# nianticlabs/simplerecon

Hardware: AMD Instinct MI355X
Metric: depth frames/sec (640x480, 7 src views, 64 planes) (higher is better)
Workload: dtype f32

## Files before the change

### include/simplerecon_hip.h

```cpp
#ifndef SIMPLERECON_HIP_H_
#define SIMPLERECON_HIP_H_

#include <stddef.h>
#include <stdint.h>

#ifdef __cplusplus
extern "C" {
#endif

#define SR_OK 0
#define SR_ERR_INVALID_ARGUMENT 1
#define SR_ERR_UNSUPPORTED 2
#define SR_ERR_WORKSPACE_TOO_SMALL 3
#define SR_ERR_HIP_BASE 1000

enum {
  SR_OPT_MLP_SPLIT = 0, SR_OPT_WINO_SPLIT, SR_OPT_WINO_XCD, SR_OPT_WINO_NT, SR_OPT_WINO_KSPLIT, SR_OPT_CONV_WINO,
  SR_OPT_CONV_TILE, SR_OPT_CONV_KSPLIT, SR_OPT_PW_NT, SR_OPT_PW_KS, SR_OPT_PT_CFG, SR_OPT_PT_KS, SR_OPT_DOT_LDS,
  SR_OPT_DOT_LDS_G, SR_OPT_DOT_LDS_CULL, SR_OPT_DOT_LDS_CAP, SR_OPT_UPSAMPLE_QUAD, SR_OPT_POOL_STREAM,
  SR_OPT_MLP_TILE,
  SR_OPT_COUNT
};
int sr_option_count(void);
const char* sr_option_name(int id);
int sr_option_id(const char* name);
int sr_option_get(int id, int* value);
int sr_option_set(int id, int value, int* previous );
int sr_option_default(int id, int* value);

int sr_abi_version(void);

const char* sr_target_arch(void);


size_t sr_volume_workspace_bytes(int B, int K, int C, int h, int w);

int sr_volume_prepare(const float* src, const float* K_src, const float* T_src_cur,
                      const float* T_cur_src, int B, int K, int C, int h, int w, void* workspace,
                      size_t workspace_bytes, void* stream);

int sr_dot_volume_sweep(const float* cur, const float* invK_cur, const float* planes, int64_t ps_b,
                        int64_t ps_d, int64_t ps_y, int64_t ps_x, int B, int K, int C, int h, int w,
                        int D, float* out_cv, int64_t cv_sb, int64_t cv_sd, int64_t cv_sp,
                        float* out_lowest, uint8_t* out_mask, void* workspace,
                        size_t workspace_bytes, void* stream);

int sr_conv3x3_wino_io_nhwc_fwd(const void* in, int64_t in_batch_stride, int in_pix_stride, const float* packed_u,
                                const float* bias, const void* residual, int64_t res_batch_stride, int res_pix_stride,
                                void* out, int64_t out_batch_stride, int out_pix_stride, int B, int H, int W, int Cin,
                                int Cout, float leaky_slope, int io_dtype, void* stream);
int sr_pw_conv_io_nhwc_fwd(const void* in, int64_t in_batch_stride, int in_pix_stride, const float* packed_w,
                           const float* bias, const void* residual, int64_t res_batch_stride, int res_pix_stride, void* out,
                           int64_t out_batch_stride, int out_pix_stride, int B, int HW, int Cin, int Cout, float act_code,
                           int io_dtype, void* stream);

size_t sr_pw_conv_tiled_workspace_bytes(int M, int Cin, int Cout);
int sr_pw_conv_tiled_plan(int M, int Cin, int Cout, int can_split, int* cfg, int* ks);
int sr_pw_conv_tiled_nhwc_fwd(const float* in, int in_pix_stride, const float* packed_w, const float* bias,
                              const float* gate, const float* residual, int res_pix_stride, float* out,
                              int out_pix_stride, int M, int HW, int Cin, int Cout, float act_code, void* workspace,
                              size_t workspace_bytes, void* stream);
int sr_pw_conv_supported(int Cin, int Cout);
int sr_pw_conv_plan(int B, int HW, int Cin, int Cout, int* nt, int* ks);
int sr_pw_conv_nhwc_fwd(const float* in, int64_t in_batch_stride, int in_pix_stride, const float* packed_w,
                        const float* bias, const float* gate, const float* residual, int64_t res_batch_stride,
                        int res_pix_stride, float* out, int64_t out_batch_stride, int out_pix_stride, int B, int HW,
                        int Cin, int Cout, float act_code, void* stream);

int sr_backproject_fwd(const float* depth, const float* invK, float* out_points, int B, int h, int w, void* stream);
int sr_project3d_fwd(const float* points, const float* K, const float* T, float* out, int B, int N, float eps,
                     void* stream);
int sr_backproject_bwd(const float* grad_points, const float* invK, float* grad_depth, int B, int h, int w, void* stream);
int sr_project3d_bwd(const float* grad_out, const float* points, const float* K, const float* T, float* grad_points, int B,
                     int N, float eps, void* stream);
int sr_pose_distance_fwd(const float* T, float* out, int n, void* stream);
int sr_camera_rays_fwd(const float* points, const float* T, float* out, int B, int N, int in_camera_frame, void* stream);

int sr_selftest_rcp(const float* x, float* out_fast, float* out_div, int n, void* stream);

int sr_dot_volume_fwd(const float* cur, const float* src, const float* K_src,
                      const float* T_src_cur, const float* invK_cur, const float* planes,
                      int64_t ps_b, int64_t ps_d, int64_t ps_y, int64_t ps_x, int B, int K, int C,
                      int h, int w, int D, float* out_cv, int64_t cv_sb, int64_t cv_sd,
                      int64_t cv_sp, float* out_lowest, uint8_t* out_mask, void* workspace,
                      size_t workspace_bytes, void* stream);

int sr_warp_features_fwd(const float* src, const float* K_src, const float* T_src_cur,
                         const float* invK_cur, const float* planes, int64_t ps_b, int64_t ps_d,
                         int64_t ps_y, int64_t ps_x, int B, int K, int C, int h, int w, int Dp,
                         float* out_world, float* out_depths, float* out_warped, float* out_mask,
                         float* out_pix, void* workspace, size_t workspace_bytes, void* stream);

size_t sr_mlp_volume_workspace_bytes(int B, int K, int C, int h, int w, int hidden);

int sr_mlp_pack_weights(const float* W1, const float* b1, const float* W2, const float* b2,
                        const float* W3, const float* b3, int hidden, int B, int K, int C, int h, int w,
                        void* workspace, size_t workspace_bytes, void* stream);

int sr_mlp_volume_sweep(const float* cur, const float* invK_cur, const float* planes, int64_t ps_b,
                        int64_t ps_d, int64_t ps_y, int64_t ps_x, float leaky_slope, int B, int K,
                        int C, int h, int w, int D, float* out_cv, int64_t cv_sb, int64_t cv_sd,
                        int64_t cv_sp, float* out_lowest, uint8_t* out_mask, void* workspace,
                        size_t workspace_bytes, void* stream);

int sr_mlp_volume_tile_shape(int h, int w, int* th, int* tw);

int sr_mlp_volume_fwd(const float* cur, const float* src, const float* K_src, const float* T_src_cur,
                      const float* T_cur_src, const float* invK_cur, const float* planes, int64_t ps_b,
                      int64_t ps_d, int64_t ps_y, int64_t ps_x, const float* W1, const float* b1,
                      const float* W2, const float* b2, const float* W3, const float* b3, int hidden,
                      float leaky_slope, int B, int K, int C, int h, int w, int D, float* out_cv,
                      int64_t cv_sb, int64_t cv_sd, int64_t cv_sp, float* out_lowest, uint8_t* out_mask,
                      int reserve_cus, void* workspace, size_t workspace_bytes, void* stream);


size_t sr_conv_packed_weight_floats(int Cout, int Cin, int ksize);

int sr_conv_pack_weights(const float* weight, int Cout, int Cin, int ksize, float* packed, void* stream);

int sr_conv2d_nhwc_fwd(const float* in, int64_t in_batch_stride, int in_pix_stride,
                       const float* packed_weight, const float* bias, const float* residual,
                       int64_t res_batch_stride, int res_pix_stride, float* out,
                       int64_t out_batch_stride, int out_pix_stride, int B, int H, int W, int Cin,
                       int Cout, int ksize, int stride, float leaky_slope, void* stream);

int sr_conv2d_replicate_nhwc_fwd(const float* in, int64_t in_batch_stride, int in_pix_stride,
                                 const float* packed_weight, const float* bias, const float* residual,
                                 int64_t res_batch_stride, int res_pix_stride, float* out,
                                 int64_t out_batch_stride, int out_pix_stride, int B, int H, int W, int Cin,
                                 int Cout, int ksize, int stride, float leaky_slope, void* stream);

#define SR_ACT_NONE (-1.0f)
#define SR_ACT_SILU (-2.0f)
int sr_conv2d_padded_nhwc_fwd(const float* in, int64_t in_batch_stride, int in_pix_stride,
                              const float* packed_weight, const float* bias, const float* residual,
                              int64_t res_batch_stride, int res_pix_stride, float* out,
                              int64_t out_batch_stride, int out_pix_stride, int B, int H, int W, int Cin,
                              int Cout, int ksize, int stride, int pad_top, int pad_left, int pad_bottom,
                              int pad_right, float leaky_slope, void* stream);

size_t sr_conv_splitk_workspace_bytes(int B, int H, int W, int Cin, int Cout, int ksize, int stride);
int sr_conv2d_splitk_nhwc_fwd(const float* in, int64_t in_batch_stride, int in_pix_stride,
                              const float* packed_weight, const float* bias, const float* residual,
                              int64_t res_batch_stride, int res_pix_stride, float* out,
                              int64_t out_batch_stride, int out_pix_stride, int B, int H, int W, int Cin,
                              int Cout, int ksize, int stride, float leaky_slope, void* workspace,
                              size_t workspace_bytes, void* stream);

size_t sr_wino_packed_weight_floats(int Cout, int Cin);
int sr_wino_pack_weights(const float* weight, int Cout, int Cin, float* packed, void* stream);
int sr_conv_prefers_wino(int B, int H, int W, int Cin, int Cout, int ksize, int stride);
int sr_conv3x3_wino_nhwc_fwd(const float* in, int64_t in_batch_stride, int in_pix_stride,
                             const float* packed_u, const float* bias, const float* residual,
                             int64_t res_batch_stride, int res_pix_stride, float* out,
                             int64_t out_batch_stride, int out_pix_stride, int B, int H, int W, int Cin,
                             int Cout, float leaky_slope, void* stream);

size_t sr_wino4_packed_weight_floats(int Cout, int Cin);
// ... 383 lines not shown
```

### simplerecon_amd/_lib.py

```python
import contextlib
import ctypes as C
import os

import torch

_HERE = os.path.dirname(os.path.abspath(__file__))
LIB_PATH = os.environ.get("SR_HIP_LIBRARY") or os.path.join(_HERE, "libsimplerecon_hip.so")
ABI_VERSION = 3

_lib = None

_p = C.c_void_p
_i = C.c_int
_i64 = C.c_int64
_f = C.c_float
_sz = C.c_size_t

SIGNATURES = {
    "sr_abi_version": (_i, []),
    "sr_option_count": (_i, []),
    "sr_option_name": (C.c_char_p, [_i]),
    "sr_option_id": (_i, [C.c_char_p]),
    "sr_option_get": (_i, [_i, C.POINTER(C.c_int)]),
    "sr_option_set": (_i, [_i, _i, C.POINTER(C.c_int)]),
    "sr_option_default": (_i, [_i, C.POINTER(C.c_int)]),
    "sr_target_arch": (C.c_char_p, []),
    "sr_volume_workspace_bytes": (_sz, [_i, _i, _i, _i, _i]),
    "sr_volume_prepare": (_i, [_p, _p, _p, _p, _i, _i, _i, _i, _i, _p, _sz, _p]),
    "sr_dot_volume_sweep": (_i, [_p, _p, _p, _i64, _i64, _i64, _i64, _i, _i, _i, _i, _i, _i,
                                 _p, _i64, _i64, _i64, _p, _p, _p, _sz, _p]),
    "sr_dot_volume_fwd": (_i, [_p, _p, _p, _p, _p, _p, _i64, _i64, _i64, _i64, _i, _i, _i, _i, _i, _i,
                               _p, _i64, _i64, _i64, _p, _p, _p, _sz, _p]),
    "sr_rgb_stem3x3s2_fwd": (_i, [_p, _i64, _i64, _i64, _i64, _p, _p, _p, _i64, _i, _i, _i, _i, _i, _i, _i, _i, _i, _f, _p]),
    "sr_se_gate2_fwd": (_i, [_p, _i, _i, _p, _p, _p, _p, _p, _p, _i, _i, _i, _p]),
    "sr_conv3x3_wino_io_nhwc_fwd": (_i, [_p, _i64, _i, _p, _p, _p, _i64, _i, _p, _i64, _i, _i, _i, _i, _i, _i, _f, _i, _p]),
    "sr_pw_conv_io_nhwc_fwd": (_i, [_p, _i64, _i, _p, _p, _p, _i64, _i, _p, _i64, _i, _i, _i, _i, _i, _f, _i, _p]),
    "sr_conv16_packed_weight_bytes": (_sz, [_i, _i, _i]),
    "sr_conv16_pack_weights": (_i, [_p, _i, _i, _i, _i, _p, _p]),
    "sr_conv16_supported": (_i, [_i, _i, _i, _i, _i, _i, _i]),
    "sr_conv16_prefers": (_i, [_i, _i, _i, _i, _i, _i, _i]),
    "sr_conv16_nhwc_fwd": (_i, [_p, _i64, _i, _p, _p, _p, _i64, _i, _p, _i64, _i, _i, _i, _i, _i, _i, _i, _i, _f, _i, _i, _p]),
    "sr_conv16_wgrad_supported": (_i, [_i, _i, _i, _i, _i, _i, _i]),
    "sr_conv16_wgrad_prefers": (_i, [_i, _i, _i, _i, _i, _i, _i]),
    "sr_conv16_wgrad_workspace_bytes": (_sz, [_i, _i, _i, _i, _i, _i, _i]),
    "sr_conv16_wgrad_nhwc": (_i, [_p, _i64, _i, _p, _i64, _i, _p, _i, _i, _i, _i, _i, _i, _i, _i, _p, _sz, _p]),
    "sr_act_bwd_bias16_workspace_bytes": (_sz, [_i64, _i]),
    "sr_act_bwd_bias16_nhwc": (_i, [_p, _i, _p, _p, _p, _i64, _i, _f, _i, _p, _sz, _p]),
    "sr_pw_conv_tiled_workspace_bytes": (_sz, [_i, _i, _i]),
    "sr_pw_conv_tiled_plan": (_i, [_i, _i, _i, _i, _p, _p]),
    "sr_pw_conv_tiled_nhwc_fwd": (_i, [_p, _i, _p, _p, _p, _p, _i, _p, _i, _i, _i, _i, _i, _f, _p, _sz, _p]),
    "sr_pw_conv_supported": (_i, [_i, _i]),
    "sr_pw_conv_plan": (_i, [_i, _i, _i, _i, _p, _p]),
    "sr_pw_conv_nhwc_fwd": (_i, [_p, _i64, _i, _p, _p, _p, _p, _i64, _i, _p, _i64, _i, _i, _i, _i, _i, _f, _p]),
    "sr_backproject_fwd": (_i, [_p, _p, _p, _i, _i, _i, _p]),
    "sr_project3d_fwd": (_i, [_p, _p, _p, _p, _i, _i, _f, _p]),
    "sr_backproject_bwd": (_i, [_p, _p, _p, _i, _i, _i, _p]),
    "sr_project3d_bwd": (_i, [_p, _p, _p, _p, _p, _i, _i, _f, _p]),
    "sr_pose_distance_fwd": (_i, [_p, _p, _i, _p]),
    "sr_camera_rays_fwd": (_i, [_p, _p, _p, _i, _i, _i, _p]),
    "sr_selftest_rcp": (_i, [_p, _p, _p, _i, _p]),
    "sr_warp_features_fwd": (_i, [_p, _p, _p, _p, _p, _i64, _i64, _i64, _i64, _i, _i, _i, _i, _i, _i,
                                  _p, _p, _p, _p, _p, _p, _sz, _p]),
    "sr_mlp_volume_workspace_bytes": (_sz, [_i, _i, _i, _i, _i, _i]),
    "sr_mlp_pack_weights": (_i, [_p, _p, _p, _p, _p, _p, _i, _i, _i, _i, _i, _i, _p, _sz, _p]),
    "sr_mlp_volume_sweep": (_i, [_p, _p, _p, _i64, _i64, _i64, _i64, _f, _i, _i, _i, _i, _i, _i,
                                 _p, _i64, _i64, _i64, _p, _p, _p, _sz, _p]),
    "sr_mlp_volume_tile_shape": (_i, [_i, _i, C.POINTER(C.c_int), C.POINTER(C.c_int)]),
    "sr_mlp_volume_fwd": (_i, [_p, _p, _p, _p, _p, _p, _p, _i64, _i64, _i64, _i64, _p, _p, _p, _p, _p, _p, _i,
                               _f, _i, _i, _i, _i, _i, _i, _p, _i64, _i64, _i64, _p, _p, _i, _p, _sz, _p]),
    "sr_conv_packed_weight_floats": (_sz, [_i, _i, _i]),
    "sr_conv_pack_weights": (_i, [_p, _i, _i, _i, _p, _p]),
    "sr_conv2d_nhwc_fwd": (_i, [_p, _i64, _i, _p, _p, _p, _i64, _i, _p, _i64, _i, _i, _i, _i, _i, _i, _i, _i, _f, _p]),
    "sr_conv2d_replicate_nhwc_fwd": (_i, [_p, _i64, _i, _p, _p, _p, _i64, _i, _p, _i64, _i, _i, _i, _i, _i, _i, _i, _i,
                                          _f, _p]),
    "sr_conv2d_padded_nhwc_fwd": (_i, [_p, _i64, _i, _p, _p, _p, _i64, _i, _p, _i64, _i, _i, _i, _i, _i, _i, _i, _i,
                                       _i, _i, _i, _i, _f, _p]),
    "sr_dwconv3x3_pool_bands": (_i, [_i]),
    "sr_dwconv3x3_nhwc_fwd": (_i, [_p, _i64, _i, _p, _p, _p, _i64, _i, _p, _i, _i, _i, _i, _i, _i, _i, _i, _i, _f,
                                   _p]),
    "sr_add_nhwc_fwd": (_i, [_p, _i64, _i, _p, _i64, _i, _p, _i64, _i, _i, _i, _i, _i, _p]),
    "sr_se_scale_nhwc_fwd": (_i, [_p, _i, _p, _p, _p, _p, _p, _p, _i64, _i, _p, _i64, _i, _p, _i, _i, _i, _i, _i,
                                  _p]),
    "sr_se_gate_fwd": (_i, [_p, _i, _i, _p, _p, _p, _p, _p, _i, _i, _i, _p]),
    "sr_scale_channels_nhwc_fwd": (_i, [_p, _i64, _i, _p, _p, _i64, _i, _i, _i, _i, _i, _p]),
    "sr_dot_volume_bwd_scratch_bytes": (_sz, [_i, _i, _i, _i, _i]),
    "sr_dot_volume_bwd": (_i, [_p, _i64, _i64, _i64, _p, _p, _p, _i64, _i64, _i64, _i64, _i, _i, _i, _i, _i, _i, _p, _p,
                               _p, _sz, _p, _sz, _p]),
    "sr_mlp_volume_bwd_scratch_bytes": (_sz, [_i, _i, _i, _i, _i, _i]),
    "sr_mlp_volume_bwd": (_i, [_p, _i64, _i64, _i64, _p, _p, _p, _i64, _i64, _i64, _i64, _p, _p, _p, _p, _p, _f, _i, _i,
                               _i, _i, _i, _i, _i, _p, _p, _p, _p, _p, _p, _p, _p, _p, _sz, _p, _sz, _p]),
    "sr_conv_wgrad_workspace_bytes": (_sz, [_i, _i, _i, _i, _i, _i, _i]),
    "sr_conv_wgrad_nhwc": (_i, [_p, _i64, _i, _p, _i64, _i, _p, _i, _i, _i, _i, _i, _i, _i, _p, _sz, _p]),
    "sr_bias_grad_nhwc": (_i, [_p, _i64, _i, _p, _i, _i, _i, _i, _p]),
    "sr_act_bwd": (_i, [_p, _p, _p, _i64, _f, _p]),
    "sr_act_bwd_bias_workspace_bytes": (_sz, [_i64, _i]),
    "sr_act_bwd_bias_nhwc": (_i, [_p, _p, _p, _p, _i64, _i, _f, _p, _sz, _p]),
    "sr_zero_stuff2x_nhwc": (_i, [_p, _i64, _i, _p, _i, _i, _i, _i, _i, _i, _p]),
    "sr_upsample2x_bwd_nhwc": (_i, [_p, _i64, _i, _p, _i64, _i, _i, _i, _i, _i, _p]),
    "sr_conv_flip_transpose_weights": (_i, [_p, _i, _i, _i, _p, _p]),
    "sr_mul_fwd": (_i, [_p, _p, _p, _i64, _p]),
    "sr_norm_workspace_bytes": (_sz, [_i, _i, _i, _i]),
    "sr_norm_stats_nhwc": (_i, [_p, _i64, _i, _i, _i, _i, _i, _p, _p, _p, _sz, _p]),
    "sr_norm_act_fwd_nhwc": (_i, [_p, _i64, _i, _p, _p, _f, _p, _p, _f, _i, _p, _i64, _i, _i, _i, _i, _p]),
    "sr_norm_act_bwd_nhwc": (_i, [_p, _i64, _i, _p, _i64, _i, _p, _p, _f, _p, _p, _f, _i, _i, _p, _i64, _i, _p, _p,
                                  _i, _i, _i, _p, _sz, _p]),
    "sr_rowsum_nhwc": (_i, [_p, _i64, _i, _p, _i64, _i, _i, _i, _i, _f, _p, _p, _sz, _p]),
    "sr_maxblurpool_bwd_workspace_bytes": (_sz, [_i, _i, _i, _i]),
    "sr_maxblurpool_bwd_nhwc": (_i, [_p, _i64, _i, _p, _i64, _i, _p, _i64, _i, _i, _i, _i, _i, _p, _sz, _p]),
    "sr_replicate_pad_nhwc_fwd": (_i, [_p, _i64, _i, _p, _i, _i, _i, _i, _i, _p]),
    "sr_replicate_pad_nhwc_bwd": (_i, [_p, _p, _i, _i, _i, _i, _i, _p]),
    "sr_im2col7x7s2_nhwc": (_i, [_p, _i64, _i64, _i64, _i64, _p, _i, _i, _i, _i, _p]),
    "sr_dwconv3x3_bwd_workspace_bytes": (_sz, [_i, _i, _i, _i]),
    "sr_dwconv3x3_bwd_nhwc": (_i, [_p, _i64, _i, _p, _i64, _i, _p, _p, _p, _i, _i, _i, _i, _i, _i, _i, _i, _i, _p, _sz,
                                   _p]),
    "sr_scale_bwd_nhwc": (_i, [_p, _i64, _i, _p, _p, _f, _p, _i, _i, _i, _p]),
    "sr_small_linear_fwd": (_i, [_p, _p, _p, _p, _p, _i, _i, _i, _f, _p]),
    "sr_small_linear_bwd": (_i, [_p, _p, _p, _p, _p, _p, _p, _i, _i, _i, _f, _p]),
    "sr_act_in_bwd": (_i, [_p, _p, _p, _i64, _f, _p]),
    "sr_add_act_fwd": (_i, [_p, _p, _p, _p, _i64, _f, _p]),
    "sr_conv_wgrad_padded_workspace_bytes": (_sz, [_i, _i, _i, _i, _i, _i]),
# ... 287 lines not shown
```

### simplerecon_amd/csrc/sr_mlp_volume.hip

```cpp
#include <stdlib.h>
#include <string.h>

#include "sr_buffer.h"
#include "sr_view.h"

#define SR_HID 128
#define SR_VIEW_SLOTS 24
#define SR_INV_FIXED 20
#define SR_PLANE_CHUNK 8

static inline int sr_mlp_steps_var(int K) { return (SR_VIEW_SLOTS / 2) * K; }
static inline int sr_mlp_steps_inv(int K) { return (SR_INV_FIXED + 3 * K + 1) / 2; }
static inline int sr_mlp_steps1(int K) { return sr_mlp_steps_var(K) + sr_mlp_steps_inv(K); }
#define SR_MLP_STEPS2 65

static inline size_t sr_mlp_packed_floats(int K) { return (size_t)(sr_mlp_steps1(K) + SR_MLP_STEPS2) * 256 + 128 + 4; }

__global__ void sr_mlp_pack_kernel(const float* __restrict__ W1, const float* __restrict__ b1,
                                   const float* __restrict__ W2, const float* __restrict__ b2,
                                   const float* __restrict__ W3, const float* __restrict__ b3,
                                   float* __restrict__ packed, int K, int C) {
  const int steps_var = (SR_VIEW_SLOTS / 2) * K;
  const int steps1 = steps_var + (SR_INV_FIXED + 3 * K + 1) / 2;
  const int Cin = C * (K + 1) + 10 * K + 4;
// ... 16 lines not shown
        else if (s == 18) col = o_dot + k;
        else if (s == 19) col = o_ang + k;
        else if (s < 23) col = o_sray + 3 * k + (s - 20);
        else col = (k == 0) ? o_d : -1;
      } else {
        const int u = 2 * (t - steps_var) + (lane >> 5);
        if (u < 16) col = o_cur + u;
        else if (u < 19) col = o_cray + (u - 16);
        else if (u == 19) col = -2;
        else if (u < SR_INV_FIXED + 3 * K) {
          const int k = (u - SR_INV_FIXED) / 3, i = (u - SR_INV_FIXED) - 3 * k;
          col = (i == 0 ? o_pd : (i == 1 ? o_rm : o_tm)) + k;
        }
      }
      v = (col >= 0) ? W1[(size_t)row * Cin + col] : (col == -2 ? b1[row] : 0.0f);
    } else if (e < (steps1 + SR_MLP_STEPS2) * 256) {
      const int e2 = e - steps1 * 256;
      const int t = e2 >> 8, lane = (e2 >> 2) & 63, mt = e2 & 3;
      const int row = 32 * mt + (lane & 31);
      if (t < 64) {
        const int m = t >> 4, r = t & 15;
        const int f = 32 * m + (r & 3) + 8 * (r >> 2) + 4 * (lane >> 5);
        v = W2[(size_t)row * SR_HID + f];
      } else {
        v = (lane < 32) ? b2[row] : 0.0f;
      }
    } else if (e < (steps1 + SR_MLP_STEPS2) * 256 + 128) {
      const int i = e - (steps1 + SR_MLP_STEPS2) * 256;
      const int half = i >> 6, mt = (i >> 4) & 3, r = i & 15;
      v = W3[32 * mt + (r & 3) + 8 * (r >> 2) + 4 * half];
    } else {
      v = b3[0];
    }
    packed[e] = v;
  }
}


struct SrMlpParams {
  const float* cur;
  const float* src_nhwc;
  const float* invK;
  const float* geom;
  const float* packed;
  SrPlanes planes;
  SrVolumeOut out;
  int B, K, h, w, D;
  int tiles;
  int tiles_x;
  int th_log2, tw_log2;
  int chunk, chunks;
  int vec_store;
  float inv_w, inv_h, slope;
};

__device__ __forceinline__ bool sr_mlp_lane_pixel(const SrMlpParams& p, int tile, int lane, int& y, int& x) {
  if (p.tiles_x) {
    const int ty = tile / p.tiles_x, tx = tile - ty * p.tiles_x;
    const int ly = (ty << p.th_log2) + (lane >> p.tw_log2);
    const int lx = (tx << p.tw_log2) + (lane & ((1 << p.tw_log2) - 1));
    y = min(ly, p.h - 1);
    x = min(lx, p.w - 1);
    return ly < p.h && lx < p.w;
  }
  const int N = p.h * p.w, pix = tile * 64 + lane;
  const int pc = min(pix, N - 1);
  y = pc / p.w;
  x = pc - y * p.w;
  return pix < N;
}

__device__ __forceinline__ void sr_swap_halves(float fa, float fb, float& bP, float& bQ) {
  auto r = __builtin_amdgcn_permlane32_swap(__float_as_uint(fa), __float_as_uint(fb), false, false);
  bP = __uint_as_float(r[0]);
  bQ = __uint_as_float(r[1]);
}

#define SR_MFMA(a, b, c) __builtin_amdgcn_mfma_f32_32x32x2f32((a), (b), (c), 0, 0, 0)

__device__ __forceinline__ void sr_l1_step(f32x16 (&acc)[2][4], const float4 wA, float fa, float fb) {
  float bP, bQ;
  sr_swap_halves(fa, fb, bP, bQ);
  acc[0][0] = SR_MFMA(wA.x, bP, acc[0][0]);
  acc[1][0] = SR_MFMA(wA.x, bQ, acc[1][0]);
  acc[0][1] = SR_MFMA(wA.y, bP, acc[0][1]);
  acc[1][1] = SR_MFMA(wA.y, bQ, acc[1][1]);
  acc[0][2] = SR_MFMA(wA.z, bP, acc[0][2]);
  acc[1][2] = SR_MFMA(wA.z, bQ, acc[1][2]);
  acc[0][3] = SR_MFMA(wA.w, bP, acc[0][3]);
  acc[1][3] = SR_MFMA(wA.w, bQ, acc[1][3]);
}

__device__ __forceinline__ void sr_l1_step_init(f32x16 (&acc)[2][4], const f32x16 (&hc)[2][4], const float4 wA,
                                                float fa, float fb) {
  float bP, bQ;
  sr_swap_halves(fa, fb, bP, bQ);
  acc[0][0] = SR_MFMA(wA.x, bP, hc[0][0]);
  acc[1][0] = SR_MFMA(wA.x, bQ, hc[1][0]);
  acc[0][1] = SR_MFMA(wA.y, bP, hc[0][1]);
  acc[1][1] = SR_MFMA(wA.y, bQ, hc[1][1]);
  acc[0][2] = SR_MFMA(wA.z, bP, hc[0][2]);
  acc[1][2] = SR_MFMA(wA.z, bQ, hc[1][2]);
  acc[0][3] = SR_MFMA(wA.w, bP, hc[0][3]);
  acc[1][3] = SR_MFMA(wA.w, bQ, hc[1][3]);
}

__device__ __forceinline__ int sr_opaque(bool flag) {
  int v = __builtin_amdgcn_readfirstlane((int)flag);
  asm volatile("" : "+s"(v));
  return v;
}

#define SR_LDS_W3_FLOATS 256

template <bool W1_LDS, bool W2_LDS>
__global__ __launch_bounds__(256, 1) void sr_mlp_volume_kernel(SrMlpParams p) {
  extern __shared__ __attribute__((aligned(16))) float lds[];
  constexpr int C = 16;
  constexpr int VS = SR_VIEW_SLOTS / 2;
  const int lane = threadIdx.x & 63;
  const int steps_var = VS * p.K;
  const int steps1 = steps_var + (SR_INV_FIXED + 3 * p.K + 1) / 2;
  const float4* gW1 = reinterpret_cast<const float4*>(p.packed);
  const float4* gW1inv = gW1 + (size_t)steps_var * 64;
  const float4* gW2 = gW1 + (size_t)steps1 * 64;
  const float* gW3 = p.packed + (size_t)(steps1 + SR_MLP_STEPS2) * 256;

  for (int i = threadIdx.x; i < 129; i += blockDim.x) lds[i] = gW3[i];
  constexpr int W2_FLOATS = W2_LDS ? SR_MLP_STEPS2 * 256 : 0;
  if (W2_LDS) {
    float4* l4 = reinterpret_cast<float4*>(lds + SR_LDS_W3_FLOATS);
    for (int i = threadIdx.x; i < SR_MLP_STEPS2 * 64; i += blockDim.x) l4[i] = gW2[i];
  }
  if (W1_LDS) {
    float4* l4 = reinterpret_cast<float4*>(lds + SR_LDS_W3_FLOATS + W2_FLOATS);
    for (int i = threadIdx.x; i < steps_var * 64; i += blockDim.x) l4[i] = gW1[i];
  }
  __syncthreads();
  const float4* W1p = W1_LDS ? reinterpret_cast<const float4*>(lds + SR_LDS_W3_FLOATS + W2_FLOATS) : gW1;

  const int N = p.h * p.w;
  const long nunits = (long)p.B * p.tiles * p.chunks;
  constexpr int WPB = 4;
  const int wid = __builtin_amdgcn_readfirstlane(threadIdx.x >> 6);
  long wave0 = (long)blockIdx.x * WPB + wid;
  long nwaves = (long)gridDim.x * WPB;
  long unit_end = nunits;
  if ((gridDim.x & 7) == 0) {
    const long u8 = (nunits + 7) / 8;
    const int xcd = blockIdx.x & 7;
    nwaves = (long)(gridDim.x >> 3) * WPB;
    wave0 = xcd * u8 + (long)(blockIdx.x >> 3) * WPB + wid;
    unit_end = min(nunits, (xcd + 1) * u8);
  }
  const int half = lane >> 5;

  const int rot = (int)max(1L, nwaves / p.chunks);
  for (long unit = wave0; unit < unit_end; unit += nwaves) {
    const long tb = unit / p.chunks;
    const int chunk = (int)((unit % p.chunks + tb / rot) % p.chunks);
    const int tile = (int)(tb % p.tiles);
    const int b = (int)(tb / p.tiles);
    const int j0 = chunk * p.chunk, j1 = min(p.D, j0 + p.chunk);
    int y, x;
    const bool in_image = sr_mlp_lane_pixel(p, tile, lane, y, x);
    const int pc = y * p.w + x;
    const int pix = in_image ? pc : -1;
    const bool active = pix >= 0;
    const float* plane_ptr = p.planes.ptr + b * p.planes.sb + y * p.planes.sy + x * p.planes.sx;
    const float* geom_b = p.geom + (size_t)b * p.K * SR_GEOM_STRIDE;
    const float* src_b = p.src_nhwc + (size_t)b * p.K * N * C;

    float cur[C];
#pragma unroll
    for (int c = 0; c < C; ++c) cur[c] = p.cur[((size_t)b * C + c) * N + pc];

    float r0, r1, r2;
    {
#pragma clang fp contract(off)
      const float* iK = p.invK + 16 * (size_t)b;
      const float px = (float)x + 0.5f, py = (float)y + 0.5f;
      r0 = iK[0] * px + iK[1] * py + iK[2];
      r1 = iK[4] * px + iK[5] * py + iK[6];
      r2 = iK[8] * px + iK[9] * py + iK[10];
    }
    float cr0, cr1, cr2, crn0, crn1, crn2;
    {
#pragma clang fp contract(off)
      const float d0 = plane_ptr[0];
      const float X0 = d0 * r0, X1 = d0 * r1, X2 = d0 * r2;
      const float cden = fmaxf(sqrtf((X0 * X0 + X1 * X1) + X2 * X2), 1e-12f);
      cr0 = X0 / cden; cr1 = X1 / cden; cr2 = X2 / cden;
      const float n1 = fmaxf(sqrtf((cr0 * cr0 + cr1 * cr1) + cr2 * cr2), 1e-5f);
      crn0 = cr0 / n1; crn1 = cr1 / n1; crn2 = cr2 / n1;
    }

    f32x16 hc[2][4];
#pragma unroll
    for (int g = 0; g < 2; ++g)
#pragma unroll
      for (int m = 0; m < 4; ++m)
#pragma unroll
        for (int r = 0; r < 16; ++r) hc[g][m][r] = 0.0f;
    {
      const float4* wi = gW1inv + lane;
#pragma unroll
      for (int t = 0; t < 8; ++t) sr_l1_step(hc, wi[t * 64], cur[2 * t], cur[2 * t + 1]);
      sr_l1_step(hc, wi[8 * 64], cr0, cr1);
      sr_l1_step(hc, wi[9 * 64], cr2, 1.0f);
      const int npose = 3 * p.K;
#pragma unroll 1
      for (int u = 0; u < npose; u += 2) {
        const int ka = u / 3, ia = u - 3 * ka, kb = (u + 1) / 3, ib = (u + 1) - 3 * kb;
// ... 187 lines not shown
        acc2[0][1] = SR_MFMA(wA.y, bP, t == 0 ? zero16 : acc2[0][1]);
        acc2[1][1] = SR_MFMA(wA.y, bQ, t == 0 ? zero16 : acc2[1][1]);
        acc2[0][2] = SR_MFMA(wA.z, bP, t == 0 ? zero16 : acc2[0][2]);
        acc2[1][2] = SR_MFMA(wA.z, bQ, t == 0 ? zero16 : acc2[1][2]);
        acc2[0][3] = SR_MFMA(wA.w, bP, t == 0 ? zero16 : acc2[0][3]);
        acc2[1][3] = SR_MFMA(wA.w, bQ, t == 0 ? zero16 : acc2[1][3]);
      }
      {
        const float4 wA = wn0;
        const float one = half ? 0.0f : 1.0f;
        acc2[0][0] = SR_MFMA(wA.x, one, acc2[0][0]);
        acc2[1][0] = SR_MFMA(wA.x, one, acc2[1][0]);
        acc2[0][1] = SR_MFMA(wA.y, one, acc2[0][1]);
        acc2[1][1] = SR_MFMA(wA.y, one, acc2[1][1]);
        acc2[0][2] = SR_MFMA(wA.z, one, acc2[0][2]);
        acc2[1][2] = SR_MFMA(wA.z, one, acc2[1][2]);
        acc2[0][3] = SR_MFMA(wA.w, one, acc2[0][3]);
        acc2[1][3] = SR_MFMA(wA.w, one, acc2[1][3]);
      }

      const float4* w3 = reinterpret_cast<const float4*>(lds + half * 64);
      sr_f2v oPQ = {0.0f, 0.0f};
      const sr_f2v slope2 = {p.slope, p.slope};
#pragma unroll
      for (int m = 0; m < 4; ++m)
#pragma unroll
        for (int q = 0; q < 4; ++q) {
          const float4 wv = w3[m * 4 + q];
          const float wr[4] = {wv.x, wv.y, wv.z, wv.w};
#pragma unroll
          for (int i = 0; i < 4; ++i) {
            const sr_f2v h2 = {acc2[0][m][4 * q + i], acc2[1][m][4 * q + i]};
            const sr_f2v s2 = slope2 * h2;
            oPQ = __builtin_elementwise_fma(sr_f2v{wr[i], wr[i]}, sr_f2v{sr_vmax(h2.x, s2.x), sr_vmax(h2.y, s2.y)}, oPQ);
          }
        }
      float oP = oPQ.x, oQ = oPQ.y;
      oP += __shfl_xor(oP, 32);
      oQ += __shfl_xor(oQ, 32);
      const float cost = (half ? oQ : oP) + lds[128];

      if (p.vec_store) {
        if (CST_LDS) lds[cst_base + (j - j0) * 64 + lane] = cost;
        else {
#pragma unroll
          for (int q = 0; q < SR_PLANE_CHUNK; ++q) cst[q] = (j - j0 == q) ? cost : cst[q];
        }
      }
      if (active) {
        if (!p.vec_store) p.out.cv[b * p.out.sb + j * p.out.sd + (int64_t)pix * p.out.sp] = cost;
        if (j == p.D - 1 && p.out.mask) p.out.mask[(size_t)b * N + pix] = (uint8_t)(any_depth && any_bounds);
      }
    }
    if (p.vec_store && active) {
      float* row = p.out.cv + b * p.out.sb + (int64_t)pix * p.out.sp + j0;
      if (CST_LDS) {
#pragma unroll
        for (int q = 0; q < SR_PLANE_CHUNK; ++q) cst[q] = lds[cst_base + q * 64 + lane];
      }
#pragma unroll
      for (int q = 0; q < SR_PLANE_CHUNK; q += 4) {
        if (j0 + q + 4 <= j1) *reinterpret_cast<float4*>(row + q) = make_float4(cst[q], cst[q + 1], cst[q + 2], cst[q + 3]);
        else {
#pragma unroll
          for (int i = 0; i < 4; ++i)
            if (j0 + q + i < j1) row[q + i] = cst[q + i];
        }
      }
    }
  }
}


template <int FMT> struct SrSplitFmt;
template <> struct SrSplitFmt<1> {
  typedef __bf16 e2 __attribute__((ext_vector_type(2)));
  typedef __bf16 e8 __attribute__((ext_vector_type(8)));
  static __device__ __forceinline__ void split(float a, float b, unsigned& hi, unsigned& lo) {
    const sr_f2v v = {a, b};
    hi = __builtin_bit_cast(unsigned, __builtin_convertvector(v, e2));
    const sr_f2v v0 = {__uint_as_float(hi << 16), __uint_as_float(hi & 0xffff0000u)};
    lo = __builtin_bit_cast(unsigned, __builtin_convertvector(v - v0, e2));
  }
  static __device__ __forceinline__ f32x16 mfma(sr_u4 a, sr_u4 b, f32x16 c) {
    return __builtin_amdgcn_mfma_f32_32x32x16_bf16(__builtin_bit_cast(e8, a), __builtin_bit_cast(e8, b), c, 0, 0, 0);
  }
};
template <> struct SrSplitFmt<2> {
  typedef _Float16 e2 __attribute__((ext_vector_type(2)));
  typedef _Float16 e8 __attribute__((ext_vector_type(8)));
  static __device__ __forceinline__ void split(float a, float b, unsigned& hi, unsigned& lo) {
    const sr_f2v v = {a, b};
    const e2 h = __builtin_convertvector(v, e2);
    hi = __builtin_bit_cast(unsigned, h);
    lo = __builtin_bit_cast(unsigned, __builtin_convertvector(v - __builtin_convertvector(h, sr_f2v), e2));
  }
  static __device__ __forceinline__ f32x16 mfma(sr_u4 a, sr_u4 b, f32x16 c) {
    return __builtin_amdgcn_mfma_f32_32x32x16_f16(__builtin_bit_cast(e8, a), __builtin_bit_cast(e8, b), c, 0, 0, 0);
  }
};

#define SR_SPL_TAB 512
#define SR_SPL_W2_WORDS 16384
#define SR_SPL_VIEW_WORDS 3072

template <int FMT>
__global__ void sr_mlp_pack_split_kernel(const float* __restrict__ W1, const float* __restrict__ b1,
                                         const float* __restrict__ W2, const float* __restrict__ b2,
                                         const float* __restrict__ W3, const float* __restrict__ b3,
                                         float* __restrict__ packed, int K, int C) {
  typedef SrSplitFmt<FMT> S;
  const int steps_var = (SR_VIEW_SLOTS / 2) * K;
  const int steps_inv = (SR_INV_FIXED + 3 * K + 1) / 2;
  const int steps1 = steps_var + steps_inv;
  const int Cin = C * (K + 1) + 10 * K + 4;
  const int o_cur = K * C, o_mask = o_cur + C, o_z = o_mask + K, o_d = o_z + K, o_dot = o_d + 1;
  const int o_ang = o_dot + K, o_cray = o_ang + K, o_sray = o_cray + 3, o_pd = o_sray + 3 * K;
  const int o_rm = o_pd + K, o_tm = o_rm + K;
  unsigned* pk = reinterpret_cast<unsigned*>(packed);
  auto var_col = [&](int k, int s) {
    if (s < 16) return k * C + s;
    if (s == 16) return o_mask + k;
// ... 308 lines not shown
      }
      if (active) {
        if (!p.vec_store) p.out.cv[b * p.out.sb + j * p.out.sd + (int64_t)pix * p.out.sp] = cost;
        if (j == p.D - 1 && p.out.mask) p.out.mask[(size_t)b * N + pix] = (uint8_t)(any_depth && any_bounds);
      }
    }
    if (p.vec_store && active) {
      float* row = p.out.cv + b * p.out.sb + (int64_t)pix * p.out.sp + j0;
#pragma unroll
      for (int q = 0; q < SR_PLANE_CHUNK; q += 4) {
        if (j0 + q + 4 <= j1) *reinterpret_cast<float4*>(row + q) = make_float4(cst[q], cst[q + 1], cst[q + 2], cst[q + 3]);
        else {
#pragma unroll
          for (int i = 0; i < 4; ++i)
            if (j0 + q + i < j1) row[q + i] = cst[q + i];
        }
      }
    }
  }
}

static int sr_mlp_split_mode() { return sr_opt(SR_OPT_MLP_SPLIT); }

__global__ void sr_argmax_planes_kernel(const float* __restrict__ cv, int64_t sb, int64_t sd, int64_t sp,
                                        SrPlanes planes, int h, int w, int D, float* __restrict__ lowest) {
  const int N = h * w;
  const int pix = blockIdx.x * blockDim.x + threadIdx.x;
  const int b = blockIdx.y;
  if (pix >= N) return;
  const int y = pix / w, x = pix - y * w;
  const float* c = cv + b * sb + (int64_t)pix * sp;
  float best = c[0];
  int bj = 0;
  int j = 1;
  for (; j + 8 <= D; j += 8) {
    float v[8];
#pragma unroll
    for (int u = 0; u < 8; ++u) v[u] = c[(int64_t)(j + u) * sd];
#pragma unroll
    for (int u = 0; u < 8; ++u)
      if (v[u] > best || (v[u] != v[u] && best == best)) { best = v[u]; bj = j + u; }
  }
  for (; j < D; ++j) {
    const float v = c[(int64_t)j * sd];
    if (v > best || (v != v && best == best)) { best = v; bj = j; }
  }
  lowest[(size_t)b * N + pix] = planes.ptr[b * planes.sb + bj * planes.sd + y * planes.sy + x * planes.sx];
}


extern "C" size_t sr_mlp_volume_workspace_bytes(int B, int K, int C, int h, int w, int hidden) {
  (void)hidden;
  if (B < 0 || K < 0) return 0;
  return sr_volume_workspace_bytes(B, K, C, h, w) + sr_align_up(sr_mlp_packed_floats(K) * sizeof(float), 256) + 256;
}

extern "C" int sr_mlp_volume_tile_shape(int h, int w, int* th, int* tw) {
  if (h <= 0 || w <= 0 || !th || !tw) return SR_ERR_INVALID_ARGUMENT;
  const int mode = sr_opt(SR_OPT_MLP_TILE);
  if (mode < 0 || mode > 4) return SR_ERR_INVALID_ARGUMENT;
  *th = 1; *tw = 64;
  if (mode >= 2) { *th = 1 << (mode - 1); *tw = 64 >> (mode - 1); }
  if (mode == 0) {
    const int64_t flat = ((int64_t)h * w + 63) / 64;
    for (int t = 8; t >= 2; t >>= 1) {
      const int64_t tiles = (int64_t)((h + t - 1) / t) * ((w + 64 / t - 1) / (64 / t));
      if (100 * tiles <= 101 * flat) { *th = t; *tw = 64 / t; break; }
    }
  }
  return SR_OK;
}

static float* sr_ws_packed(void* workspace, int B, int K, int C, int h, int w) {
  return (float*)sr_align_up((size_t)workspace + sr_volume_workspace_bytes(B, K, C, h, w), 256);
}

static int sr_mlp_volume_sweep_reserved(const float* cur, const float* invK_cur, const float* planes, int64_t ps_b,
                                        int64_t ps_d, int64_t ps_y, int64_t ps_x, float leaky_slope, int B, int K,
                                        int C, int h, int w, int D, float* out_cv, int64_t cv_sb, int64_t cv_sd,
                                        int64_t cv_sp, float* out_lowest, uint8_t* out_mask, int reserve_cus,
                                        void* workspace, size_t workspace_bytes, void* stream_) {
  if (B < 0 || K <= 0 || C <= 0 || h <= 0 || w <= 0 || D <= 0) return SR_ERR_INVALID_ARGUMENT;
  if (B == 0) return SR_OK;
  if (!cur || !invK_cur || !planes || !out_cv || !workspace) return SR_ERR_INVALID_ARGUMENT;
  if (C != 16) return SR_ERR_UNSUPPORTED;
  if (!(leaky_slope > 0.0f && leaky_slope < 1.0f)) return SR_ERR_UNSUPPORTED;
  if (workspace_bytes < sr_mlp_volume_workspace_bytes(B, K, C, h, w, SR_HID)) return SR_ERR_WORKSPACE_TOO_SMALL;
  hipStream_t stream = (hipStream_t)stream_;
  const int N = h * w;

  SrMlpParams p;
  p.cur = cur; p.src_nhwc = sr_ws_src_nhwc(workspace, B, K); p.invK = invK_cur; p.geom = sr_ws_geom(workspace);
  p.packed = sr_ws_packed(workspace, B, K, C, h, w);
  p.planes = {planes, ps_b, ps_d, ps_y, ps_x};
  p.out = {out_cv, cv_sb, cv_sd, cv_sp, out_lowest, out_mask};
  p.B = B; p.K = K; p.h = h; p.w = w; p.D = D;
  int th, tw;
  if (sr_mlp_volume_tile_shape(h, w, &th, &tw)) return SR_ERR_INVALID_ARGUMENT;
  p.th_log2 = __builtin_ctz(th); p.tw_log2 = __builtin_ctz(tw);
  p.tiles_x = th == 1 ? 0 : (w + tw - 1) / tw;
  p.tiles = th == 1 ? (N + 63) / 64 : p.tiles_x * ((h + th - 1) / th);
  p.inv_w = (float)(1.0 / (double)w);
  p.inv_h = (float)(1.0 / (double)h);
  p.slope = leaky_slope;

  int cus = sr_device_cus();
  if (reserve_cus > 0 && cus - reserve_cus >= 8) cus -= reserve_cus;
  const long waves = 4L * cus;
  double best_cost = 1e30;
  int best = 1;
  for (int c = SR_PLANE_CHUNK; c >= 1; c >>= 1) {
    const long units = (long)B * p.tiles * ((D + c - 1) / c);
    const long rounds = (units + waves - 1) / waves;
    const double cost = (double)rounds * (c * 1192.0 + 168.0);
    if (cost < best_cost) { best_cost = cost; best = c; }
  }
  p.chunk = best;
  p.chunks = (D + best - 1) / best;
  p.vec_store = (cv_sd == 1) && (p.chunk % 4 == 0) && sr_rows_aligned(out_cv, cv_sb, cv_sp, 15, 4);
  const long nunits = (long)B * p.tiles * p.chunks;
  const int blocks = (int)((nunits + 3) / 4 < cus ? (nunits + 3) / 4 : cus);
  const size_t w3_bytes = SR_LDS_W3_FLOATS * sizeof(float);
  const size_t w1_bytes = (size_t)sr_mlp_steps_var(K) * 1024;
  const size_t w2_bytes = (size_t)SR_MLP_STEPS2 * 1024;
  const size_t lds_max = 160 * 1024;
  const int split = sr_mlp_split_mode();
  if (split < 0) return SR_ERR_INVALID_ARGUMENT;
  if (split) {
    const size_t bytes = ((size_t)SR_SPL_TAB + SR_SPL_W2_WORDS + (size_t)K * SR_SPL_VIEW_WORDS) * 4;
    if (bytes > lds_max) return SR_ERR_UNSUPPORTED;
    const void* fn = split == 1 ? (const void*)sr_mlp_volume_split_kernel<1> : (const void*)sr_mlp_volume_split_kernel<2>;
    if (hipError_t e = sr_allow_lds(fn, bytes)) return sr_hip_rc(e);
    if (split == 1) hipLaunchKernelGGL((sr_mlp_volume_split_kernel<1>), dim3(blocks), dim3(256), bytes, stream, p);
    else hipLaunchKernelGGL((sr_mlp_volume_split_kernel<2>), dim3(blocks), dim3(256), bytes, stream, p);
    int rc = sr_hip_rc(hipGetLastError());
    if (rc) return rc;
    if (out_lowest) rc = sr_launch_argmax_planes(out_cv, cv_sb, cv_sd, cv_sp, p.planes, B, h, w, D, out_lowest, stream);
    return rc;
  }
#define SR_MLP_LAUNCH(L1, L2, BYTES)                                                                              \
  {                                                                                                               \
           \
    if (hipError_t e = sr_allow_lds((const void*)sr_mlp_volume_kernel<L1, L2>, (BYTES))) return sr_hip_rc(e);     \
    hipLaunchKernelGGL((sr_mlp_volume_kernel<L1, L2>), dim3(blocks), dim3(256), (BYTES), stream, p);              \
  }
  if (w1_bytes + w2_bytes + w3_bytes <= lds_max) SR_MLP_LAUNCH(true, true, w1_bytes + w2_bytes + w3_bytes)
  else if (w1_bytes + w3_bytes <= lds_max) SR_MLP_LAUNCH(true, false, w1_bytes + w3_bytes)
  else SR_MLP_LAUNCH(false, true, w2_bytes + w3_bytes + 4 * SR_PLANE_CHUNK * 64 * sizeof(float))
#undef SR_MLP_LAUNCH
  int rc = sr_hip_rc(hipGetLastError());
  if (rc) return rc;
  if (out_lowest) rc = sr_launch_argmax_planes(out_cv, cv_sb, cv_sd, cv_sp, p.planes, B, h, w, D, out_lowest, stream);
  return rc;
}

extern "C" int sr_mlp_volume_sweep(const float* cur, const float* invK_cur, const float* planes, int64_t ps_b,
                                   int64_t ps_d, int64_t ps_y, int64_t ps_x, float leaky_slope, int B, int K,
                                   int C, int h, int w, int D, float* out_cv, int64_t cv_sb, int64_t cv_sd,
                                   int64_t cv_sp, float* out_lowest, uint8_t* out_mask, void* workspace,
                                   size_t workspace_bytes, void* stream_) {
  return sr_mlp_volume_sweep_reserved(cur, invK_cur, planes, ps_b, ps_d, ps_y, ps_x, leaky_slope, B, K, C, h, w, D, out_cv,
                                      cv_sb, cv_sd, cv_sp, out_lowest, out_mask, 0, workspace, workspace_bytes, stream_);
}

int sr_launch_argmax_planes(const float* cv, int64_t sb, int64_t sd, int64_t sp, SrPlanes planes, int B, int h, int w,
                            int D, float* lowest, hipStream_t stream) {
  hipLaunchKernelGGL(sr_argmax_planes_kernel, dim3((h * w + 63) / 64, B), dim3(64), 0, stream, cv, sb, sd, sp,
                     planes, h, w, D, lowest);
  return sr_hip_rc(hipGetLastError());
}

extern "C" int sr_mlp_pack_weights(const float* W1, const float* b1, const float* W2, const float* b2,
                                   const float* W3, const float* b3, int hidden, int B, int K, int C, int h, int w,
                                   void* workspace, size_t workspace_bytes, void* stream_) {
  if (!W1 || !b1 || !W2 || !b2 || !W3 || !b3 || !workspace || K <= 0) return SR_ERR_INVALID_ARGUMENT;
  if (hidden != SR_HID || C != 16) return SR_ERR_UNSUPPORTED;
  if (workspace_bytes < sr_mlp_volume_workspace_bytes(B, K, C, h, w, hidden)) return SR_ERR_WORKSPACE_TOO_SMALL;
  const int split = sr_mlp_split_mode();
  if (split < 0) return SR_ERR_INVALID_ARGUMENT;
  float* packed = sr_ws_packed(workspace, B, K, C, h, w);
  if (split == 1) hipLaunchKernelGGL((sr_mlp_pack_split_kernel<1>), dim3(64), dim3(256), 0, (hipStream_t)stream_, W1, b1, W2, b2, W3, b3, packed, K, C);
  else if (split == 2) hipLaunchKernelGGL((sr_mlp_pack_split_kernel<2>), dim3(64), dim3(256), 0, (hipStream_t)stream_, W1, b1, W2, b2, W3, b3, packed, K, C);
  else hipLaunchKernelGGL(sr_mlp_pack_kernel, dim3(64), dim3(256), 0, (hipStream_t)stream_, W1, b1, W2, b2, W3, b3, packed, K, C);
  return sr_hip_rc(hipGetLastError());
}

extern "C" int sr_mlp_volume_fwd(const float* cur, const float* src, const float* K_src, const float* T_src_cur,
                                 const float* T_cur_src, const float* invK_cur, const float* planes, int64_t ps_b,
                                 int64_t ps_d, int64_t ps_y, int64_t ps_x, const float* W1, const float* b1,
                                 const float* W2, const float* b2, const float* W3, const float* b3, int hidden,
                                 float leaky_slope, int B, int K, int C, int h, int w, int D, float* out_cv,
                                 int64_t cv_sb, int64_t cv_sd, int64_t cv_sp, float* out_lowest, uint8_t* out_mask,
                                 int reserve_cus, void* workspace, size_t workspace_bytes, void* stream_) {
  if (B < 0 || K <= 0 || C <= 0 || h <= 0 || w <= 0 || D <= 0 || reserve_cus < 0) return SR_ERR_INVALID_ARGUMENT;
  if (B == 0) return SR_OK;
  if (!T_cur_src) return SR_ERR_INVALID_ARGUMENT;
  if (hidden != SR_HID || C != 16) return SR_ERR_UNSUPPORTED;
// ... 10 lines not shown
```

### simplerecon_amd/csrc/sr_options.hip

```cpp
#include <atomic>
#include <map>
#include <mutex>
#include <utility>
#include <stdlib.h>
#include <string.h>

#include "sr_common.h"

namespace {

struct OptDef { const char* name; int dflt; int kind; };
const OptDef kDefs[SR_OPT_COUNT] = {
    {"SR_MLP_SPLIT", 0, 1},       {"SR_WINO_SPLIT", 0, 1},     {"SR_WINO_XCD", 1, 0},        {"SR_WINO_NT", 0, 0},
    {"SR_WINO_KSPLIT", 0, 0},     {"SR_CONV_WINO", 1, 0},      {"SR_CONV_TILE", 0, 0},       {"SR_CONV_KSPLIT", 1, 0},
    {"SR_PW_NT", 0, 0},           {"SR_PW_KS", 0, 0},          {"SR_PT_CFG", -1, 0},         {"SR_PT_KS", 0, 0},
    {"SR_DOT_LDS", 1, 0},         {"SR_DOT_LDS_G", 0, 0},      {"SR_DOT_LDS_CULL", 1, 0},    {"SR_DOT_LDS_CAP", 634, 0},
    {"SR_UPSAMPLE_QUAD", 1, 0},   {"SR_POOL_STREAM", 1, 0},    {"SR_MLP_TILE", 0, 2},
};
std::atomic<int> g_val[SR_OPT_COUNT];
std::once_flag g_once;

int parse(const OptDef& d, const char* e) {
  if (d.kind == 1) {
    if (!e || !*e || !strcmp(e, "0") || !strcmp(e, "off") || !strcmp(e, "fp32")) return 0;
    if (!strcmp(e, "bf16")) return 1;
    if (!strcmp(e, "f16") || !strcmp(e, "fp16")) return 2;
    return -1;
  }
  if (d.kind == 2) {
    static const char* const names[] = {"auto", "flat", "2x32", "4x16", "8x8"};
    if (!e || !*e) return d.dflt;
    for (int i = 0; i < 5; ++i)
      if (!strcmp(e, names[i])) return i;
    return -1;
  }
  return (e && *e) ? atoi(e) : d.dflt;
}

void init() {
  for (int i = 0; i < SR_OPT_COUNT; ++i) {
    const char* e = getenv(kDefs[i].name);
    g_val[i].store(e ? parse(kDefs[i], e) : kDefs[i].dflt, std::memory_order_relaxed);
  }
}

}

int sr_opt(int id) {
  std::call_once(g_once, init);
  return g_val[id].load(std::memory_order_relaxed);
}

extern "C" int sr_option_count(void) { return SR_OPT_COUNT; }

extern "C" const char* sr_option_name(int id) { return (id >= 0 && id < SR_OPT_COUNT) ? kDefs[id].name : nullptr; }

extern "C" int sr_option_id(const char* name) {
  if (!name) return -1;
  for (int i = 0; i < SR_OPT_COUNT; ++i)
    if (!strcmp(kDefs[i].name, name)) return i;
  return -1;
}

extern "C" int sr_option_get(int id, int* value) {
  if (id < 0 || id >= SR_OPT_COUNT || !value) return SR_ERR_INVALID_ARGUMENT;
  *value = sr_opt(id);
  return SR_OK;
}

extern "C" int sr_option_set(int id, int value, int* previous) {
// ... 39 lines not shown
```

Before: 328.3.

## Add atomic work-queue scheduling for MLP cost-volume kernel

```diff
diff --git a/include/simplerecon_hip.h b/include/simplerecon_hip.h
--- a/include/simplerecon_hip.h
+++ b/include/simplerecon_hip.h
@@ -18,7 +18,7 @@
   SR_OPT_MLP_SPLIT = 0, SR_OPT_WINO_SPLIT, SR_OPT_WINO_XCD, SR_OPT_WINO_NT, SR_OPT_WINO_KSPLIT, SR_OPT_CONV_WINO,
   SR_OPT_CONV_TILE, SR_OPT_CONV_KSPLIT, SR_OPT_PW_NT, SR_OPT_PW_KS, SR_OPT_PT_CFG, SR_OPT_PT_KS, SR_OPT_DOT_LDS,
   SR_OPT_DOT_LDS_G, SR_OPT_DOT_LDS_CULL, SR_OPT_DOT_LDS_CAP, SR_OPT_UPSAMPLE_QUAD, SR_OPT_POOL_STREAM,
-  SR_OPT_MLP_TILE,
+  SR_OPT_MLP_TILE, SR_OPT_MLP_QUEUE,
   SR_OPT_COUNT
 };
 int sr_option_count(void);
@@ -104,6 +104,9 @@
                         size_t workspace_bytes, void* stream);
 
 int sr_mlp_volume_tile_shape(int h, int w, int* th, int* tw);
+
+int sr_mlp_volume_queue_band(int pairs, int queues, int q, int* pair0, int* count);
+int sr_mlp_volume_queue_item(int item, int pair0, int count, int chunks, int block, int* pair, int* chunk);
 
 int sr_mlp_volume_fwd(const float* cur, const float* src, const float* K_src, const float* T_src_cur,
                       const float* T_cur_src, const float* invK_cur, const float* planes, int64_t ps_b,
diff --git a/simplerecon_amd/_lib.py b/simplerecon_amd/_lib.py
--- a/simplerecon_amd/_lib.py
+++ b/simplerecon_amd/_lib.py
@@ -66,6 +66,8 @@
     "sr_mlp_volume_sweep": (_i, [_p, _p, _p, _i64, _i64, _i64, _i64, _f, _i, _i, _i, _i, _i, _i,
                                  _p, _i64, _i64, _i64, _p, _p, _p, _sz, _p]),
     "sr_mlp_volume_tile_shape": (_i, [_i, _i, C.POINTER(C.c_int), C.POINTER(C.c_int)]),
+    "sr_mlp_volume_queue_band": (_i, [_i, _i, _i, C.POINTER(C.c_int), C.POINTER(C.c_int)]),
+    "sr_mlp_volume_queue_item": (_i, [_i, _i, _i, _i, _i, C.POINTER(C.c_int), C.POINTER(C.c_int)]),
     "sr_mlp_volume_fwd": (_i, [_p, _p, _p, _p, _p, _p, _p, _i64, _i64, _i64, _i64, _p, _p, _p, _p, _p, _p, _i,
                                _f, _i, _i, _i, _i, _i, _i, _p, _i64, _i64, _i64, _p, _p, _i, _p, _sz, _p]),
     "sr_conv_packed_weight_floats": (_sz, [_i, _i, _i]),
diff --git a/simplerecon_amd/csrc/sr_mlp_volume.hip b/simplerecon_amd/csrc/sr_mlp_volume.hip
--- a/simplerecon_amd/csrc/sr_mlp_volume.hip
+++ b/simplerecon_amd/csrc/sr_mlp_volume.hip
@@ -92,7 +92,29 @@
   int chunk, chunks;
   int vec_store;
   float inv_w, inv_h, slope;
+  unsigned* queue;
+  int qblock;
 };
+
+#define SR_MLP_QUEUE_STRIDE 8
+#define SR_MLP_QUEUE_BLOCK 64
+__host__ __device__ __forceinline__ void sr_mlp_queue_band(int pairs, int queues, int q, int& pair0, int& count) {
+  const int per = (pairs + queues - 1) / queues;
+  const long first = (long)q * per;
+  pair0 = first < pairs ? (int)first : pairs;
+  count = (pairs - pair0 < per) ? pairs - pair0 : per;
+}
+__global__ void sr_mlp_queue_zero_kernel(unsigned* queue) { queue[threadIdx.x] = 0u; }
+__host__ __device__ __forceinline__ void sr_mlp_queue_item(unsigned i, int pair0, int count, int chunks, int qblock,
+                                                           int& pair, int& chunk) {
+  const unsigned per_block = (unsigned)qblock * (unsigned)chunks;
+  const unsigned blk = i / per_block, r = i - blk * per_block;
+  const unsigned first = blk * (unsigned)qblock;
+  const unsigned nb = (unsigned)count - first < (unsigned)qblock ? (unsigned)count - first : (unsigned)qblock;
+  const unsigned rank = r / nb;
+  chunk = chunks - 1 - (int)rank;
+  pair = pair0 + (int)(first + (r - rank * nb));
+}
 
 __device__ __forceinline__ bool sr_mlp_lane_pixel(const SrMlpParams& p, int tile, int lane, int& y, int& x) {
   if (p.tiles_x) {
@@ -153,7 +175,7 @@
 
 #define SR_LDS_W3_FLOATS 256
 
-template <bool W1_LDS, bool W2_LDS>
+template <bool W1_LDS, bool W2_LDS, bool QUEUED>
 __global__ __launch_bounds__(256, 1) void sr_mlp_volume_kernel(SrMlpParams p) {
   extern __shared__ __attribute__((aligned(16))) float lds[];
   constexpr int C = 16;
@@ -186,7 +208,7 @@
   long wave0 = (long)blockIdx.x * WPB + wid;
   long nwaves = (long)gridDim.x * WPB;
   long unit_end = nunits;
-  if ((gridDim.x & 7) == 0) {
+  if (!QUEUED && (gridDim.x & 7) == 0) {
     const long u8 = (nunits + 7) / 8;
     const int xcd = blockIdx.x & 7;
     nwaves = (long)(gridDim.x >> 3) * WPB;
@@ -196,9 +218,42 @@
   const int half = lane >> 5;
 
   const int rot = (int)max(1L, nwaves / p.chunks);
-  for (long unit = wave0; unit < unit_end; unit += nwaves) {
-    const long tb = unit / p.chunks;
-    const int chunk = (int)((unit % p.chunks + tb / rot) % p.chunks);
+  const int queues = (gridDim.x & 7) == 0 ? 8 : 1;
+  int q = blockIdx.x & (queues - 1);
+  int qleft = queues;
+  unsigned item = 0;
+  auto take = [&]() -> unsigned {
+    unsigned* ctr = p.queue + SR_MLP_QUEUE_STRIDE * q;
+    unsigned got = 0;
+    if (lane == 0) got = atomicAdd(ctr, 1u);
+    return got;
+  };
+  auto broadcast = [](unsigned got) -> unsigned {
+    unsigned v = __builtin_amdgcn_readfirstlane(got);
+    asm volatile("" : "+s"(v));
+    return v;
+  };
+  if (QUEUED) item = broadcast(take());
+  for (long unit = wave0;; unit += nwaves) {
+    long tb;
+    int chunk;
+    if (QUEUED) {
+      int pair0, count;
+      for (;;) {
+        sr_mlp_queue_band(p.B * p.tiles, queues, q, pair0, count);
+        if (item < (unsigned)count * (unsigned)p.chunks || --qleft == 0) break;
+        q = (q + 1) & (queues - 1);
+        item = broadcast(take());
+      }
+      if (qleft == 0) break;
+      int pair;
+      sr_mlp_queue_item(item, pair0, count, p.chunks, p.qblock, pair, chunk);
+      tb = pair;
+    } else {
+      if (unit >= unit_end) break;
+      tb = unit / p.chunks;
+      chunk = (int)((unit % p.chunks + tb / rot) % p.chunks);
+    }
     const int tile = (int)(tb % p.tiles);
     const int b = (int)(tb / p.tiles);
     const int j0 = chunk * p.chunk, j1 = min(p.D, j0 + p.chunk);
@@ -492,6 +547,8 @@
         if (j == p.D - 1 && p.out.mask) p.out.mask[(size_t)b * N + pix] = (uint8_t)(any_depth && any_bounds);
       }
     }
+    unsigned next = 0;
+    if (QUEUED) next = take();
     if (p.vec_store && active) {
       float* row = p.out.cv + b * p.out.sb + (int64_t)pix * p.out.sp + j0;
       if (CST_LDS) {
@@ -508,6 +565,7 @@
         }
       }
     }
+    if (QUEUED) item = broadcast(next);
   }
 }
 
@@ -922,7 +980,21 @@
 extern "C" size_t sr_mlp_volume_workspace_bytes(int B, int K, int C, int h, int w, int hidden) {
   (void)hidden;
   if (B < 0 || K < 0) return 0;
-  return sr_volume_workspace_bytes(B, K, C, h, w) + sr_align_up(sr_mlp_packed_floats(K) * sizeof(float), 256) + 256;
+  return sr_volume_workspace_bytes(B, K, C, h, w) + sr_align_up(sr_mlp_packed_floats(K) * sizeof(float), 256) + 256 + 256;
+}
+
+extern "C" int sr_mlp_volume_queue_band(int pairs, int queues, int q, int* pair0, int* count) {
+  if (pairs <= 0 || (queues != 1 && queues != 8) || q < 0 || q >= queues || !pair0 || !count) return SR_ERR_INVALID_ARGUMENT;
+  sr_mlp_queue_band(pairs, queues, q, *pair0, *count);
+  return SR_OK;
+}
+
+extern "C" int sr_mlp_volume_queue_item(int item, int pair0, int count, int chunks, int block, int* pair, int* chunk) {
+  if (pair0 < 0 || count <= 0 || chunks <= 0 || block <= 0 || !pair || !chunk) return SR_ERR_INVALID_ARGUMENT;
+  if (block > count) block = count;
+  if (item < 0 || (int64_t)item >= (int64_t)count * chunks) return SR_ERR_INVALID_ARGUMENT;
+  sr_mlp_queue_item((unsigned)item, pair0, count, chunks, block, *pair, *chunk);
+  return SR_OK;
 }
 
 extern "C" int sr_mlp_volume_tile_shape(int h, int w, int* th, int* tw) {
@@ -943,6 +1015,10 @@
 
 static float* sr_ws_packed(void* workspace, int B, int K, int C, int h, int w) {
   return (float*)sr_align_up((size_t)workspace + sr_volume_workspace_bytes(B, K, C, h, w), 256);
+}
+
+static unsigned* sr_ws_queue(void* workspace, int B, int K, int C, int h, int w) {
+  return (unsigned*)((char*)sr_ws_packed(workspace, B, K, C, h, w) + sr_align_up(sr_mlp_packed_floats(K) * sizeof(float), 256));
 }
 
 static int sr_mlp_volume_sweep_reserved(const float* cur, const float* invK_cur, const float* planes, int64_t ps_b,
@@ -973,6 +1049,7 @@
   p.inv_w = (float)(1.0 / (double)w);
   p.inv_h = (float)(1.0 / (double)h);
   p.slope = leaky_slope;
+  p.queue = nullptr; p.qblock = 1;
 
   int cus = sr_device_cus();
   if (reserve_cus > 0 && cus - reserve_cus >= 8) cus -= reserve_cus;
@@ -1008,11 +1085,27 @@
     if (out_lowest) rc = sr_launch_argmax_planes(out_cv, cv_sb, cv_sd, cv_sp, p.planes, B, h, w, D, out_lowest, stream);
     return rc;
   }
+  const int qmode = sr_opt(SR_OPT_MLP_QUEUE);
+  if (qmode < 0) return SR_ERR_INVALID_ARGUMENT;
+  if (qmode > 0 && nunits < (1L << 31)) {
+    p.queue = sr_ws_queue(workspace, B, K, C, h, w);
+    hipLaunchKernelGGL(sr_mlp_queue_zero_kernel, dim3(1), dim3(SR_MLP_QUEUE_STRIDE * 8), 0, stream, p.queue);
+    if (int rc = sr_hip_rc(hipGetLastError())) return rc;
+    const int queues = (blocks & 7) ? 1 : 8;
+    const int band = (int)((nunits / p.chunks + queues - 1) / queues);
+    const int block = qmode == 1 ? SR_MLP_QUEUE_BLOCK : qmode;
+    p.qblock = block > band ? band : block;
+  }
 #define SR_MLP_LAUNCH(L1, L2, BYTES)                                                                              \
   {                                                                                                               \
            \
-    if (hipError_t e = sr_allow_lds((const void*)sr_mlp_volume_kernel<L1, L2>, (BYTES))) return sr_hip_rc(e);     \
-    hipLaunchKernelGGL((sr_mlp_volume_kernel<L1, L2>), dim3(blocks), dim3(256), (BYTES), stream, p);              \
+    if (p.queue) {                                                                                                \
+      if (hipError_t e = sr_allow_lds((const void*)sr_mlp_volume_kernel<L1, L2, true>, (BYTES))) return sr_hip_rc(e); \
+      hipLaunchKernelGGL((sr_mlp_volume_kernel<L1, L2, true>), dim3(blocks), dim3(256), (BYTES), stream, p);      \
+    } else {                                                                                                      \
+      if (hipError_t e = sr_allow_lds((const void*)sr_mlp_volume_kernel<L1, L2, false>, (BYTES))) return sr_hip_rc(e); \
+      hipLaunchKernelGGL((sr_mlp_volume_kernel<L1, L2, false>), dim3(blocks), dim3(256), (BYTES), stream, p);     \
+    }                                                                                                             \
   }
   if (w1_bytes + w2_bytes + w3_bytes <= lds_max) SR_MLP_LAUNCH(true, true, w1_bytes + w2_bytes + w3_bytes)
   else if (w1_bytes + w3_bytes <= lds_max) SR_MLP_LAUNCH(true, false, w1_bytes + w3_bytes)
diff --git a/simplerecon_amd/csrc/sr_options.hip b/simplerecon_amd/csrc/sr_options.hip
--- a/simplerecon_amd/csrc/sr_options.hip
+++ b/simplerecon_amd/csrc/sr_options.hip
@@ -16,6 +16,7 @@
     {"SR_PW_NT", 0, 0},           {"SR_PW_KS", 0, 0},          {"SR_PT_CFG", -1, 0},         {"SR_PT_KS", 0, 0},
     {"SR_DOT_LDS", 1, 0},         {"SR_DOT_LDS_G", 0, 0},      {"SR_DOT_LDS_CULL", 1, 0},    {"SR_DOT_LDS_CAP", 634, 0},
     {"SR_UPSAMPLE_QUAD", 1, 0},   {"SR_POOL_STREAM", 1, 0},    {"SR_MLP_TILE", 0, 2},
+    {"SR_MLP_QUEUE", 1, 0},
 };
 std::atomic<int> g_val[SR_OPT_COUNT];
 std::once_flag g_once;
```

New measurement: 330.9 (median of 6 runs). Within noise of the previous version (+0.8%).
